# kchmck/p25rx

Measured on AMD Instinct MI355X. Metric: IQ Msamples/s through FM-demod+C4FM slice, higher is better.
Workload: dtype f32

## Files before the change

### p25rx_amd/csrc/p25fe_api.hip

```cpp
#include "p25fe_kernels.hip"

#include <hip/hip_ext.h>
#include <math.h>
#include <stdio.h>
#include <stdlib.h>
#include <string.h>

#include <algorithm>
#include <array>
#include <chrono>
#include <new>
#include <utility>
#include <string>
#include <vector>

#include "p25fe_jit.h"

using namespace p25k;

namespace {

constexpr size_t BBPAD = 256;
constexpr size_t SHARD_HALO = 2560;
static_assert(SHARD_HALO >= (size_t)(DEC * (PLPAD + CLK_L + 160) + TMAX) && 160 >= TMAX + TMAX - 1 && SHARD_HALO % 8 == 0, "shard halo");
// ... 204 lines not shown
    bool on = false;
    int level = 1;
    std::vector<hipEvent_t> ev;
    std::vector<uint8_t> mask;
    uint64_t calls = 0, seq = 0;
    int slot = -1;
    void begin()
    {
        if (on && level == 3 && (seq++ % PROF_SAMPLE) != 0) { slot = -1; return; }
        slot = on ? (int)(calls++ % PROF_RING) : -1;
        if (slot >= 0) mask[(size_t)slot] = 0;
    }
    void end() { slot = -1; }
    void mark(int idx, hipStream_t st, bool ext_events)
    {
        if (slot < 0 || (idx > 1 && level != 1) || (idx <= 1 && ext_events)) return;
        if (hipEventRecord(ev[(size_t)slot * 5 + idx], st) == hipSuccess) mask[(size_t)slot] |= (uint8_t)(1u << idx);
    }
    void k1_events(bool ext_events, hipEvent_t* e0, hipEvent_t* e1)
    {
        *e0 = *e1 = nullptr;
        if (slot < 0 || !ext_events) return;
        *e0 = ev[(size_t)slot * 5 + 0]; *e1 = ev[(size_t)slot * 5 + 1];
        mask[(size_t)slot] |= 3u;
    }
};

constexpr size_t WIN_PARITY = 2, WIN_RING = 4;
struct WinSlot {
    hipEvent_t h2d_begin = nullptr, h2d_end = nullptr;
    hipEvent_t comp_begin = nullptr, comp_end = nullptr;
    hipEvent_t on_host = nullptr;
    std::array<hipEvent_t*, 5> all() { return {&h2d_begin, &h2d_end, &comp_begin, &comp_end, &on_host}; }
};
struct Windows {
    DevBuf buf[WIN_PARITY], dib[WIN_PARITY], res, anc;
    PinBuf stage[WIN_PARITY], out;
    hipStream_t cs = nullptr, os = nullptr;
    WinSlot slot[WIN_RING];
    WinSlot& of(size_t k) { return slot[k % WIN_RING]; }
    hipError_t ensure()
    {
        if (cs) return hipSuccess;
        hipError_t e = hipStreamCreateWithFlags(&cs, hipStreamNonBlocking);
        if (e == hipSuccess) e = hipStreamCreateWithFlags(&os, hipStreamNonBlocking);
        for (WinSlot& s : slot) for (hipEvent_t* x : s.all()) if (e == hipSuccess) e = hipEventCreate(x);
        return e;
    }
};

}

struct p25fe {
    p25fe_config_t cfg;
    int C = 1, n_cu = 256;
    Taps taps;
    int k1_p = 5;
    int variant = P25FE_VARIANT_BUILTIN;
    bool dflt = true;
    bool long_taps = false;
    int phase = P25FE_DECIM_PHASE;
    int n_avg = BOX;
    bool u8_lut_mode = false;
    float u8_scale = 0.0f, u8_offset = 0.0f;
    int track = 0;
    bool causal_ok = false;
    long look = 0;
    bool ext_events = true;
    int rx_cus = 0;
    int run_depth = 2;
    int sh_depth = MAX_LANES;

    int last_hip = 0;
    DevBuf d_taps;
    hipModule_t jit_mod = nullptr;
    hipFunction_t jit_fn[2][3] = {{nullptr, nullptr, nullptr}, {nullptr, nullptr, nullptr}};
    hipStream_t stream = nullptr, rx_stream = nullptr;
    const long* rs_idx = nullptr; size_t rs_n = 0, rs_stride = 0;
    Lane lanes[MAX_LANES];
    int cur = 0, lane_q[MAX_LANES - 1] = {1, 2, 3};
    Lane& lane() { return lanes[cur]; }
    RxScratch& rx() { return lanes[cur].s; }
    const RxScratch& rx() const { return lanes[cur].s; }
    DevBuf power_partial, chunk_cnt, evrec, evnext, evoff;
    unsigned long long ev_seq = 0;
    PinBuf hin, hbb, hout;
    unsigned chunk_seq = 0;
    Windows win; StreamState state; Prof prof; ShardCtx sh;
};

struct PlanarGeo {
    size_t n_tiles, n_blocks;
    explicit PlanarGeo(size_t n_bb)
    {
        n_tiles = (n_bb + TS - 1) / TS;
        if (n_tiles == 0) n_tiles = 1;
        n_blocks = (size_t)TWORDS * n_tiles + 6;
    }
    size_t floats() const { return n_blocks * PL_BLK; }
    size_t words() const { return n_blocks * SPS; }
};

constexpr size_t MAX_RANGE_BB = (size_t)0x7ff00000u * 10u;
static inline bool position_refused(uint64_t pos) { return pos >= P25FE_MAX_POSITION; }

struct Resolved {
    Taps taps;
    bool long_taps;
    bool lut_affine;
    float u8_scale, u8_offset;
    bool dflt;
};

static inline bool finite_f(float v) { return v - v == 0.0f; }
static inline bool same_bits(float a, float b) { return memcmp(&a, &b, sizeof a) == 0; }

static bool lut_is_affine(const float* lut, float sc, float of)
{
    for (int b = 0; b < 256; ++b)
        if (!same_bits(lut[b], fmaf((float)b, sc, of))) return false;
    return true;
}

static int resolve_config(const p25fe_config_t* cfg, Resolved* r)
{
    if (cfg->abi_version != P25FE_ABI_VERSION || cfg->n_decim_taps < 1 || cfg->n_decim_taps > P25FE_MAX_TAPS || cfg->n_chan_taps < 1 ||
        cfg->n_chan_taps > P25FE_MAX_TAPS || (cfg->symbol_clock != P25FE_CLOCK_FIXED && cfg->symbol_clock != P25FE_CLOCK_TRACKING && cfg->symbol_clock != P25FE_CLOCK_TRACKING_RESLICE &&
         cfg->symbol_clock != (P25FE_CLOCK_TRACKING_RESLICE | P25FE_CLOCK_CAUSAL_OK)) ||
        cfg->specialize < P25FE_SPECIALIZE_OFF || cfg->specialize > P25FE_SPECIALIZE_FORCE || cfg->decim_phase < 0 || cfg->decim_phase >= DEC ||
        cfg->n_avg_taps < 1 || cfg->n_avg_taps > P25FE_MAX_TAPS)
        return P25FE_ERR_ARG;
    memset(&r->taps, 0, sizeof r->taps);
    r->taps.n_avg = cfg->n_avg_taps;
    r->taps.avg_uniform = 1;
    for (int k = 0; k < cfg->n_avg_taps; ++k) {
        if (!finite_f(cfg->avg_taps[k])) return P25FE_ERR_ARG;
        r->taps.avg[k] = cfg->avg_taps[k];
        if (!same_bits(cfg->avg_taps[k], cfg->avg_taps[0])) r->taps.avg_uniform = 0;
    }
    for (int k = 0; k < cfg->n_decim_taps; ++k) { if (!finite_f(cfg->decim_taps[k])) return P25FE_ERR_ARG; r->taps.dec[k] = cfg->decim_taps[k]; }
    for (int k = 0; k < cfg->n_chan_taps; ++k) { if (!finite_f(cfg->chan_taps[k])) return P25FE_ERR_ARG; r->taps.ch[k] = cfg->chan_taps[k]; }
    r->long_taps = cfg->n_decim_taps > P25FE_T1 || cfg->n_chan_taps > P25FE_T2;
    if (cfg->fm_gain != 0.0f) {
        if (!finite_f(cfg->fm_gain)) return P25FE_ERR_ARG;
        r->taps.fm_gain = cfg->fm_gain;
    } else {
        if (cfg->fm_deviation_hz == 0 || cfg->fm_sample_rate_hz == 0) return P25FE_ERR_ARG;
        r->taps.fm_gain = (float)((double)cfg->fm_sample_rate_hz / (2.0 * M_PI * (double)cfg->fm_deviation_hz));
    }
    if (cfg->u8_lut_valid) {
        for (int b = 0; b < 256; ++b) { if (!finite_f(cfg->u8_lut[b])) return P25FE_ERR_ARG; r->taps.lut[b] = cfg->u8_lut[b]; }
        const float* L = r->taps.lut;
        const float cand[3][2] = {{cfg->u8_scale, cfg->u8_offset}, {L[1] - L[0], L[0]},
                                  {(float)(((double)L[255] - (double)L[0]) / 255.0), L[0]}};
        r->lut_affine = false;
        for (int c = 0; c < 3 && !r->lut_affine; ++c)
            if (finite_f(cand[c][0]) && finite_f(cand[c][1]) && lut_is_affine(L, cand[c][0], cand[c][1])) {
                r->lut_affine = true; r->u8_scale = cand[c][0]; r->u8_offset = cand[c][1];
            }
        if (!r->lut_affine) r->u8_scale = r->u8_offset = 0.0f;
    } else {
        if (!finite_f(cfg->u8_scale) || !finite_f(cfg->u8_offset)) return P25FE_ERR_ARG;
        r->lut_affine = true; r->u8_scale = cfg->u8_scale; r->u8_offset = cfg->u8_offset;
        for (int b = 0; b < 256; ++b) r->taps.lut[b] = fmaf((float)b, cfg->u8_scale, cfg->u8_offset);
    }
    Taps def;
    memset(&def, 0, sizeof def);
// ... 583 lines not shown

static int launch_planarize(p25fe_t* h, const float* d_bb, size_t bb_stride, size_t n_hist_bb, size_t n_bb, hipStream_t st)
{
    const PlanarGeo g(n_bb);
    PlanarizeArgs a;
    a.bb = d_bb; a.bb_stride = (long)bb_stride; a.n_hist = (long)n_hist_bb; a.n = (long)n_bb;
    a.f = h->rx().pl_f.get(); a.f_ch = (long)g.floats();
    a.bits = h->rx().pl_bits.get(); a.bits_ch = (long)g.words(); a.n_blocks = (long)g.n_blocks;
    a.shift = (int)h->look;
    hipLaunchKernelGGL(k_planarize, dim3((unsigned)((g.n_blocks + 1) / 2), (unsigned)h->C), dim3(WV * SPS), 0, st, a);
    HIPCHK(h, hipGetLastError());
    return P25FE_OK;
}

static int launch_detect(p25fe_t* h, const RecvCall& rc)
{
    DetArgs d;
    d.head_flag = nullptr; d.head_seq = 0u; d.head_tile_max = -1; d.head_err = nullptr;
    if (rc.wait_head) {
        d.head_flag = h->sh.flag.as<unsigned>(); d.head_seq = h->sh.seq; d.head_tile_max = h->sh.head_tile_max;
        d.head_err = h->sh.flag.as<unsigned>() + SH_FLAG_ERR;
    }
    view_planes(h, rc.range, &d); view_tiles(h, &d); view_general(h, &d);
    d.n_tiles = n_tiles_of(rc.range); d.opt = rc.opt;
    const dim3 grid((unsigned)d.n_tiles, (unsigned)h->C);
    if (rc.gen) hipLaunchKernelGGL(k_detect<true>, grid, dim3(WV), 0, rc.stream, d);
    else hipLaunchKernelGGL(k_detect<false>, grid, dim3(WV), 0, rc.stream, d);
    HIPCHK(h, hipGetLastError());
    return P25FE_OK;
}

enum ScanStep { SCAN_WHOLE, SCAN_RANGE, SCAN_TILES_G };
static int launch_scan(p25fe_t* h, const RecvCall& rc, ScanStep step, hipEvent_t ev_done)
{
    const dim3 grid = step == SCAN_RANGE ? dim3((unsigned)h->C) : dim3((unsigned)n_groups_of(n_tiles_of(rc.range)), (unsigned)h->C);
    if (rc.gen) {
        ScanArgsG c;
        view_scan(h, rc, &c);
        c.gsum = h->rx().gsum.get(); c.outs = h->rx().gouts.get(); c.gsg = h->rx().gsg.get(); c.gpg = h->rx().gpg.get();
        c.track = h->track;
        launch_ev(step == SCAN_WHOLE ? k_scan_tiles_g : step == SCAN_RANGE ? k_range_scan_g : k_scan_g_groups, grid, dim3(WV), 0, rc.stream,
                  nullptr, ev_done, c);
    } else {
        ScanArgs c;
        view_scan(h, rc, &c);
        c.tsum = h->rx().tsum.get(); c.outs = h->rx().outs.get(); c.gagg = h->rx().gagg.get(); c.gpre = h->rx().gpre.get();
        launch_ev(step == SCAN_WHOLE ? k_scan_tiles : k_range_scan, grid, dim3(WV), 0, rc.stream, nullptr, ev_done, c);
    }
    HIPCHK(h, hipGetLastError());
    return P25FE_OK;
}

static int launch_slice(p25fe_t* h, const RecvCall& rc)
{
    SliceArgs l;
    view_planes(h, rc.range, &l); view_tiles(h, &l); view_dest(rc.range, rc.dest, &l);
    l.n_tiles = n_tiles_of(rc.range); l.outs = h->rx().outs.get(); l.gpre = h->rx().gpre.get(); l.dibits2 = rc.dest.dibits2;
    if (rc.fix) l.fix = *rc.fix; else memset(&l.fix, 0, sizeof l.fix);
    launch_ev(k_slice, dim3((unsigned)l.n_tiles + (rc.fix ? 1u : 0u), (unsigned)h->C), dim3(WV), 0, rc.stream, nullptr, rc.ev_done, l);
    HIPCHK(h, hipGetLastError());
    return P25FE_OK;
}

static int launch_slice_g(p25fe_t* h, const RecvCall& rc)
{
    SliceArgsG l;
    view_planes(h, rc.range, &l); view_general(h, &l); view_dest(rc.range, rc.dest, &l);
    l.n_tiles = n_tiles_of(rc.range); l.outs = h->rx().gouts.get(); l.recs = h->rx().recs.get();
    l.track = h->track; l.dibits2 = rc.dest.dibits2;
    launch_ev(k_slice_g, dim3((unsigned)l.n_tiles, (unsigned)h->C), dim3(WV), 0, rc.stream, nullptr, rc.ev_done, l);
    HIPCHK(h, hipGetLastError());
    return P25FE_OK;
}

static int launch_slice_by_detection(p25fe_t* h, const RecvCall& rc)
{
    const size_t C = (size_t)h->C, n_bb = rc.range.n_bb;
    const int n_tiles = n_tiles_of(rc.range);
    hipStream_t st = rc.stream;
    size_t cap_ev = (size_t)n_tiles * EVCAP;
    const size_t bound = n_bb / (size_t)(W + 1) + (size_t)n_tiles + 8;
    if (bound < cap_ev) cap_ev = bound;
    const size_t stride = cap_ev + 2;
    HIPCHK(h, h->evrec.ensure(C * stride * sizeof(EvRec)));
    HIPCHK(h, h->evoff.ensure(C * (stride + 1) * sizeof(unsigned long long)));
    {
        const void* before = h->evnext.p;
        HIPCHK(h, h->evnext.ensure(C * stride * sizeof(EvNext)));
        if (h->evnext.p != before) HIPCHK(h, hipMemsetAsync(h->evnext.p, 0, h->evnext.cap, st));
    }
    EvArgs e;
    view_planes(h, rc.range, &e); view_general(h, &e); view_dest(rc.range, rc.dest, &e);
    e.n_tiles = n_tiles; e.outs = h->rx().gouts.get();
    e.rec = h->evrec.as<EvRec>(); e.nxt = h->evnext.as<EvNext>(); e.off = h->evoff.as<unsigned long long>();
    e.ev_stride = (long)stride; e.seq = ++h->ev_seq; e.result = rc.dest.result;
    hipLaunchKernelGGL(k_ev_collect, dim3((unsigned)n_tiles, (unsigned)h->C), dim3(WV), 0, st, e);
    HIPCHK(h, hipGetLastError());
    hipLaunchKernelGGL(k_ev_count, dim3((unsigned)(n_tiles < 1024 ? n_tiles : 1024), (unsigned)h->C), dim3(WV), 0, st, e);
    HIPCHK(h, hipGetLastError());
    hipLaunchKernelGGL(k_ev_scan, dim3((unsigned)h->C), dim3(WV), 0, st, e);
    HIPCHK(h, hipGetLastError());
    const size_t max_dibits = n_bb / (SPS - 1) + (size_t)n_tiles + 64;
    const size_t lim = rc.dest.dibit_stride < max_dibits ? rc.dest.dibit_stride : max_dibits;
    launch_ev(k_ev_slice, dim3((unsigned)((lim + WV * 4 - 1) / (WV * 4)), (unsigned)h->C), dim3(WV), 0, st, nullptr, rc.ev_done, e);
    HIPCHK(h, hipGetLastError());
    return P25FE_OK;
}

static int launch_recv(p25fe_t* h, const RecvCall& rc)
{
    const int n_tiles = n_tiles_of(rc.range);
    const bool detect = rc.detect && n_tiles != 0, slice = rc.slice && n_tiles != 0, scan = rc.fix == nullptr;
    hipStream_t st = rc.stream;
    int e = detect ? launch_detect(h, rc) : P25FE_OK;
    if (e) return e;
    h->prof.mark(2, st, h->ext_events);
    if (scan && (e = launch_scan(h, rc, detect ? SCAN_WHOLE : SCAN_RANGE, slice ? nullptr : rc.ev_done)) != P25FE_OK) return e;
    h->prof.mark(3, st, h->ext_events);
    if (slice) {
        if (!rc.gen) e = launch_slice(h, rc);
        else if ((e = launch_scan(h, rc, SCAN_TILES_G, nullptr)) == P25FE_OK) e = rc.reslice ? launch_slice_by_detection(h, rc) : launch_slice_g(h, rc);
        if (e) return e;
    }
    if (rc.ev_done && !scan && !slice) HIPCHK(h, hipEventRecord(rc.ev_done, st));
    h->prof.mark(4, st, h->ext_events);
    return P25FE_OK;
}

static int launch_k1_planar(p25fe_t* h, K1Launch& k, hipEvent_t k1_done, hipStream_t waiter)
{
    h->prof.mark(0, k.stream, h->ext_events);
    bool attached = false;
    if (p25fe_n_baseband_h(h, k.abs0, k.n)) {
        h->prof.k1_events(h->ext_events, &k.ev0, &k.ev1);
        if (k1_done && h->ext_events) {
            if (k.ev1) k1_done = k.ev1;
            else k.ev1 = k1_done;
            attached = true;
        }
        k.planar = true;
        if (int rc = launch_k1(h, k)) return rc;
    }
    if (k1_done) {
        if (!attached) HIPCHK(h, hipEventRecord(k1_done, k.stream));
        HIPCHK(h, hipStreamWaitEvent(waiter, k1_done, 0));
    }
    return P25FE_OK;
}

static int launch_planar_recv(p25fe_t* h, K1Launch& k, const RecvCall& rc, hipEvent_t k1_done = nullptr)
{
    if (int e = launch_k1_planar(h, k, k1_done, rc.stream)) return e;
    if (rc.range.n_bb) h->prof.mark(1, k.stream, h->ext_events);
    return launch_recv(h, rc);
}

static inline bool piecewise_refused(const p25fe_t* h) { return h->track == P25FE_CLOCK_TRACKING_RESLICE && !h->causal_ok; }

static WideConv wide_conv_of(const p25fe_t* h)
{
    WideConv cv;
    cv.scale = h->u8_scale; cv.offset = h->u8_offset;
    cv.lut = h->u8_lut_mode ? h->d_taps.as<Taps>()->lut : nullptr;
    return cv;
}
static inline bool wide_fmt_known(int fmt) { return fmt == P25FE_FMT_CF32 || fmt == P25FE_FMT_S16 || fmt == P25FE_FMT_U8; }
static inline int wide_o0(uint64_t abs0) { return (int)((PD - 1 + PD - abs0 % PD) % PD); }

static int launch_k0(p25fe_t* h, const void* d_iq, int fmt, size_t ch_stride, size_t n_hist, size_t n, uint64_t abs0,
                     float* d_out, size_t out_stride, hipStream_t st)
{
    if (!d_iq || !d_out || position_refused(abs0)) return P25FE_ERR_ARG;
    if ((reinterpret_cast<uintptr_t>(d_iq) & 15u) != 0 || (h->C > 1 && ch_stride % fmt_stride_unit(fmt) != 0)) return P25FE_ERR_ARG;
    HIPCHK(h, hipSetDevice(h->cfg.device));
    const size_t n_out = p25fe_n_predecim(abs0, n);
    if (n_out == 0) return P25FE_OK;
    K0Args a;
    a.x = static_cast<const float*>(d_iq); a.ch_stride = (long)ch_stride; a.n_hist = (long)n_hist; a.n_new = (long)n;
    a.o0 = wide_o0(abs0);
    a.y = d_out; a.y_stride = (long)out_stride; a.n_out = (long)n_out;
    const size_t per_wg = (size_t)K0_SUB * K0_SUBS;
    const dim3 grid((unsigned)((n_out + per_wg - 1) / per_wg), (unsigned)h->C);
    const WideConv cv = wide_conv_of(h);
    if (fmt == P25FE_FMT_CF32) hipLaunchKernelGGL(k_predecim, grid, dim3(WV), 0, st, a);
    else if (fmt == P25FE_FMT_S16) hipLaunchKernelGGL((k_predecim_fmt<P25FE_FMT_S16, false>), grid, dim3(WV), 0, st, a, cv);
    else if (cv.lut) hipLaunchKernelGGL((k_predecim_fmt<P25FE_FMT_U8, true>), grid, dim3(WV), 0, st, a, cv);
    else hipLaunchKernelGGL((k_predecim_fmt<P25FE_FMT_U8, false>), grid, dim3(WV), 0, st, a, cv);
// ... 1571 lines not shown
```

### p25rx_amd/csrc/p25fe_recv.hip

```cpp
#ifndef __HIPCC_RTC__
#include <hip/hip_runtime.h>
#include <stdint.h>
#endif

namespace p25k {

constexpr int W = P25FE_PEAK_W;
constexpr int SPS = P25FE_SPS;
constexpr int NSYN = P25FE_SYNC_DIBITS;
constexpr int SYNC_SPAN = P25FE_SYNC_SPAN;
constexpr int HIST_BB = SYNC_SPAN + 2 * W;
static_assert(SPS == SPS_ && PLPAD >= HIST_BB + P25FE_CLK_LOOKAHEAD, "planar layout matches the receiver");

constexpr int TSYM = 768;
constexpr int TS = TSYM * SPS;
constexpr int TWORDS = TSYM / 32;
constexpr int EVCAP = TS / (W + 1) + 8;
constexpr unsigned SYNC_NEG_MASK = ~P25FE_SYNC_SIGN_MASK & 0xffffffu;
constexpr int SCREEN_MAX_MISMATCH = 4;

struct Planar {
    const float* f;
    long f_ch;
    const uint32_t* bits;
// ... 1432 lines not shown
                } else {
                    const int e = (int)(i - T0) + PL_BLK;
                    if (track) {
                        const float* w = CI + 4 * (q & (P25FE_CLK_PHASES - 1));
                        v = w[0] * sample_at(e - 1);
                        v = __builtin_fmaf(w[1], sample_at(e), v);
                        v = __builtin_fmaf(w[2], sample_at(e + 1), v);
                        v = __builtin_fmaf(w[3], sample_at(e + 2), v);
                    } else {
                        v = sample_at(e);
                    }
                }
                if (rank >= 0 && rank + idx < room) {
                    const unsigned char db = slice_dibit(v, h, m, l);
                    dst[idx] = db;
                    if (out2) out2[rank + idx] = db;
                }
            }
        }
        return count;
    };

    int rank = 0;
    if (valid) rank += emit(so.s, so.D, so.N, T0, g.pre_end1 ? T0 + (long)g.pre_end1 - 1 : TE, hi, mid, lo, 0);
    unsigned eg = 0u, eg_prev = 0u;
    int ev_prev = 0;
    for (int k = 0; k < n_ev; ++k) {
        const int evk = ev_at(k, eg);
        const long ek = T0 + evk, sk = ek - W;
        int D, N;
        if (k == 0) clock_period(track, ((g.n_det_flags >> 16) & G_FIRST_TRACKS) && valid, so.s, so.f, sk, frac3(eg >> 16), D, N);
        else clock_period(track, ((eg >> 15) & 1u) != 0, T0 + ev_prev - W, frac3(eg_prev >> 16), sk, frac3(eg >> 16), D, N);
        float h, m, l;
        if (k < EVTHR_N) {
            h = rdl_f(el.th, 3 * k); m = rdl_f(el.th, 3 * k + 1); l = rdl_f(el.th, 3 * k + 2);
        } else {
            float v[NSYN];
            sync_gather(f, t0 + evk - W + PLPAD, v);
            sync_thresholds(v, h, m, l);
        }
        if (lane == 0 && a.sync_pos && (long)(so.event_off + k) < a.sync_stride) {
            a.sync_pos[(size_t)ch * a.sync_stride + so.event_off + k] = sk;
            a.sync_dibit[(size_t)ch * a.sync_stride + so.event_off + k] = so.dibit_off + (unsigned long long)rank;
        }
        rank += emit(sk, D, N, ek + 1, T0 + (long)(eg & 0x7fffu), h, m, l, rank);
        ev_prev = evk; eg_prev = eg;
    }
}
__global__ __launch_bounds__(WV, 4) void k_slice_g(SliceArgsG a) { slice_g_item(a, (int)blockIdx.x, (int)blockIdx.y); }
#endif

struct EvRec {
    long s;
    long g_lo, g_hi;
    int Db, Nb;
    int D2, N2;
    unsigned flags;
    float hi, mid, lo;
    int pad_;
};
static_assert(sizeof(EvRec) == 64, "EvRec layout");
struct EvNext { long pos; unsigned long long seq; };
constexpr unsigned EV_USABLE = 1u, EV_OPEN = 2u, EV_VALID = 4u;
__host__ __device__ inline long clock_J_off(long x, int D, int N, int off)
{
    const long num = x * (long)N - (long)off - 1;
    return num < 0 ? 0 : num / (long)D;
}

struct EvArgs {
    Planar pl;
    long n, abs0;
    int n_tiles;
    const ScanOutG* outs;
    const TileSumG* gsum;
    const uint16_t* evl;
    const uint32_t* evg;
    const float* evthr;
    const p25fe_anchor_t* anchor_in;
    EvRec* rec;
    EvNext* nxt;
    unsigned long long* off;
    long ev_stride;
    unsigned long long seq;
    p25fe_result_t* result;
    uint8_t* dibits;
    long dibit_stride;
    int64_t* sync_pos;
    uint64_t* sync_dibit;
    long sync_stride;
};

#ifndef P25FE_JIT
__device__ __forceinline__ void ev_collect_item(const EvArgs& a, const int tile, const int ch)
{
    const int lane = threadIdx.x;
    const long t0 = (long)tile * TS;
    const int tn = a.n - t0 < TS ? (int)(a.n - t0) : TS;
    const ScanOutG so = a.outs[(size_t)ch * a.n_tiles + tile];
    const TileSumG g = a.gsum[(size_t)ch * a.n_tiles + tile];
    const int n_ev = (int)(g.n_det_flags & 0xffffu);
    const long T0 = a.abs0 + t0;
    EvRec* rec = a.rec + (size_t)ch * a.ev_stride;
    EvNext* nxt = a.nxt + (size_t)ch * a.ev_stride;
    p25fe_anchor_t Ain;
    Ain.valid = 0; Ain.s = 0; Ain.hi = Ain.mid = Ain.lo = 0.f; Ain.period_d = SPS; Ain.period_n = 1;
    if (a.anchor_in) Ain = a.anchor_in[ch];
    const bool carry_valid = so.src >= 0 || (so.src == -1 && Ain.valid != 0);
    if (tile == 0 && lane == 0) {
        EvRec r;
        r.s = Ain.s; r.g_lo = a.abs0; r.g_hi = a.abs0 + a.n;
        const bool ok = clock_plausible(Ain.period_d, Ain.period_n);
        r.Db = ok ? Ain.period_d : SPS; r.Nb = ok ? Ain.period_n : 1; r.D2 = r.Db; r.N2 = r.Nb;
        r.flags = EV_USABLE | EV_OPEN | (Ain.valid ? EV_VALID : 0u);
        r.hi = Ain.hi; r.mid = Ain.mid; r.lo = Ain.lo; r.pad_ = 0;
        rec[0] = r;
    }
    if (!g.pre_end1) return;
    if (lane == 0 && carry_valid) {
        EvNext x; x.pos = T0 + (long)g.pre_end1 - 1; x.seq = a.seq;
        nxt[so.event_off] = x;
    }
    if (n_ev == 0) return;
    const uint16_t* evl = a.evl + ((size_t)ch * a.n_tiles + tile) * EVCAP;
    const uint32_t* evg = a.evg + ((size_t)ch * a.n_tiles + tile) * EVCAP;
    const float* f = a.pl.f + (size_t)ch * a.pl.f_ch;
    const float* eth = a.evthr + ((size_t)ch * a.n_tiles + tile) * (EVTHR_N * 3);
    for (int k0 = 0; k0 < n_ev; k0 += WV) {
        const int k = k0 + lane;
        if (k < n_ev) {
            const unsigned eg = evg[k];
            const long ek = T0 + evl[k], sk = ek - W;
            const unsigned eg_p = k ? evg[k - 1] : 0u;
            const long s_p = k ? T0 + evl[k - 1] - W : 0;
            EvRec r;
            bool us;
            if (k == 0) clock_period(true, ((g.n_det_flags >> 16) & G_FIRST_TRACKS) && carry_valid, so.s, so.f, sk, frac3(eg >> 16), r.Db, r.Nb, &us);
            else clock_period(true, ((eg >> 15) & 1u) != 0, s_p, frac3(eg_p >> 16), sk, frac3(eg >> 16), r.Db, r.Nb, &us);
            r.s = sk; r.g_lo = ek + 1; r.g_hi = T0 + (long)(eg & 0x7fffu);
            r.D2 = r.Db; r.N2 = r.Nb;
            r.flags = EV_VALID | (us ? EV_USABLE : 0u) | ((k == n_ev - 1 && (int)(eg & 0x7fffu) == tn) ? EV_OPEN : 0u) | (((eg >> 16) & 7u) << 8);
            r.hi = r.mid = r.lo = 0.f; r.pad_ = 0;
            EvRec* dst = rec + 1 + so.event_off + k;
            if (k < EVTHR_N) {
                r.hi = eth[3 * k]; r.mid = eth[3 * k + 1]; r.lo = eth[3 * k + 2];
                *dst = r;
            } else {
                dst->s = r.s; dst->g_lo = r.g_lo; dst->g_hi = r.g_hi; dst->Db = r.Db; dst->Nb = r.Nb; dst->D2 = r.D2; dst->N2 = r.N2;
                dst->flags = r.flags; dst->pad_ = 0;
            }
        }
    }
    for (int k = EVTHR_N; k < n_ev; ++k) {
        float v[NSYN], h, m, l;
        sync_gather(f, t0 + (int)evl[k] - W + PLPAD, v);
        sync_thresholds(v, h, m, l);
        if (lane == 0) { EvRec* r = rec + 1 + so.event_off + k; r->hi = h; r->mid = m; r->lo = l; }
    }
}
__global__ __launch_bounds__(WV, 4) void k_ev_collect(EvArgs a) { ev_collect_item(a, (int)blockIdx.x, (int)blockIdx.y); }

__global__ __launch_bounds__(WV, 4) void k_ev_count(EvArgs a)
{
    const int lane = threadIdx.x, ch = blockIdx.y;
    EvRec* rec = a.rec + (size_t)ch * a.ev_stride;
    const EvNext* nxt = a.nxt + (size_t)ch * a.ev_stride;
    const long n_e = (long)a.result[ch].n_sync + 1;
    const long range_end = a.abs0 + a.n;
    for (long e = (long)blockIdx.x * WV + lane; e < n_e; e += (long)gridDim.x * WV) {
        const EvRec r = rec[e];
        unsigned cnt = 0u;
        long jlo = 1;
        if (r.flags & EV_VALID) {
            int D = r.Db, N = r.Nb;
            if (!(r.flags & EV_USABLE) && e + 1 < n_e) {
                if (rec[e + 1].flags & EV_USABLE) { D = rec[e + 1].Db; N = rec[e + 1].Nb; }
            }
            long ghi = r.g_hi;
            if (r.flags & EV_OPEN) {
                const EvNext x = nxt[e];
                ghi = x.seq == a.seq ? x.pos : range_end;
            }
            if (N == 1) { D *= 4; N = 4; }
            const int off = frac3(r.flags >> 8) * (N / 4);
            long glo = r.g_lo < r.s + W + 1 ? r.s + W + 1 : r.g_lo;
            const long j0 = clock_J_off(glo - r.s, D, N, off);
            long c = ghi > glo ? clock_J_off(ghi - r.s, D, N, off) - j0 : 0;
            cnt = (unsigned)(c < 0 ? 0 : (c > 0x7fffffffL ? 0x7fffffffL : c));
            jlo = j0 + 1;
            rec[e].D2 = D; rec[e].N2 = N; rec[e].g_hi = ghi;
        }
        rec[e].g_lo = jlo;
        rec[e].pad_ = (int)cnt;
    }
}

constexpr int EVC_PER = 16;
__global__ __launch_bounds__(WV) void k_ev_scan(EvArgs a)
{
    const int lane = threadIdx.x, ch = blockIdx.x;
    const EvRec* rec = a.rec + (size_t)ch * a.ev_stride;
    unsigned long long* off = a.off + (size_t)ch * (a.ev_stride + 1);
    const long n_e = (long)a.result[ch].n_sync + 1;
    unsigned long long c_base = 0ull;
    for (long c0 = 0; c0 < n_e; c0 += (long)WV * EVC_PER) {
        unsigned cnt[EVC_PER];
        unsigned long long mine = 0;
#pragma unroll
        for (int q = 0; q < EVC_PER; ++q) {
            const long e = c0 + (long)lane * EVC_PER + q;
            cnt[q] = e < n_e ? (unsigned)rec[e].pad_ : 0u;
            mine += cnt[q];
        }
        const unsigned long long incl = wave_incl_sum64(mine, lane);
        unsigned long long o = c_base + incl - mine;
#pragma unroll
        for (int q = 0; q < EVC_PER; ++q) {
            const long e = c0 + (long)lane * EVC_PER + q;
            if (e < n_e) {
                off[e] = o;
                if (e >= 1 && a.sync_pos && e - 1 < a.sync_stride) {
                    a.sync_pos[(size_t)ch * a.sync_stride + e - 1] = rec[e].s;
                    a.sync_dibit[(size_t)ch * a.sync_stride + e - 1] = o;
                }
                o += cnt[q];
            }
        }
        c_base += __shfl(incl, WV - 1, 64);
    }
    if (lane == 0) {
        off[n_e] = c_base;
        p25fe_result_t r = a.result[ch];
        r.n_dibits = c_base;
        r.n_dibits_after_first = n_e >= 2 ? c_base - off[1] : 0;
        a.result[ch] = r;
    }
}

__global__ __launch_bounds__(WV, 4) void k_ev_slice(EvArgs a)
{
    __shared__ float CI[P25FE_CLK_PHASES * 4];
    const int lane = threadIdx.x, ch = blockIdx.y;
    const EvRec* rec = a.rec + (size_t)ch * a.ev_stride;
    const unsigned long long* off = a.off + (size_t)ch * (a.ev_stride + 1);
    const long n_e = (long)a.result[ch].n_sync + 1;
    const unsigned long long total = off[n_e];
    const unsigned long long g0 = (unsigned long long)blockIdx.x * (WV * 4);
    if (g0 >= total) return;
    for (int k = lane; k < P25FE_CLK_PHASES * 4; k += WV) CI[k] = P25FE_CLK_INTERP[k];
    phase_sync();
    const float* f = a.pl.f + (size_t)ch * a.pl.f_ch;
    uint8_t* out = a.dibits + (size_t)ch * a.dibit_stride;
    long e0 = 0;
    {
        long hi_ = n_e;
        while (hi_ - e0 > 1) {
            const long mid_ = (e0 + hi_) >> 1;
            if (off[mid_] <= g0) e0 = mid_; else hi_ = mid_;
        }
    }
    long lo_ = e0;
#pragma unroll
    for (int q = 0; q < 4; ++q) {
        const unsigned long long gi = g0 + (unsigned long long)(q * WV + lane);
        if (gi < total && (long)gi < a.dibit_stride) {
            while (lo_ + 1 < n_e && off[lo_ + 1] <= gi) ++lo_;
            const EvRec r = rec[lo_];
            const long j = r.g_lo + (long)(gi - off[lo_]);
            const long num = j * (long)r.D2 + (long)(frac3(r.flags >> 8) * (r.N2 / 4));
            const long qu = num / r.N2;
            const long i = r.s + qu;
            const int ph = (int)((((unsigned)(num - qu * r.N2) * (unsigned)P25FE_CLK_PHASES) / (unsigned)r.N2) & (unsigned)(P25FE_CLK_PHASES - 1));
            if (i < a.abs0 || i >= a.abs0 + a.n) { out[gi] = 0; continue; }
            const long p = i - a.abs0 + PLPAD;
            float b[4];
#pragma unroll
            for (int tq = 0; tq < 4; ++tq) {
                const long pp = p - 1 + tq;
                const long sy = pp / SPS;
                b[tq] = f[planar_index(sy, (int)(pp - sy * SPS))];
            }
            const float* w = CI + 4 * ph;
            float v = w[0] * b[0];
            v = __builtin_fmaf(w[1], b[1], v);
            v = __builtin_fmaf(w[2], b[2], v);
            v = __builtin_fmaf(w[3], b[3], v);
            out[gi] = slice_dibit(v, r.hi, r.mid, r.lo);
        }
    }
}
#endif

constexpr int TAILN = 256;

struct ChunkRecvArgs {
    Planar pl;
    long n;
    long abs0;
    TileRec* recs;
    unsigned long long* tsum;
    uint16_t* evl;
    float* evthr;
    const p25fe_anchor_t* anchor_in;
    p25fe_result_t* result;
    uint8_t* dibits;
    long dibit_stride;
    int64_t* sync_pos;
    uint64_t* sync_dibit;
    long sync_stride;
    float* tail;
    int look;
    unsigned long long n_baseband;
    unsigned* done;
    unsigned seq;
};

__device__ __forceinline__ void wave_global_sync() { __builtin_amdgcn_fence(__ATOMIC_SEQ_CST, "workgroup"); }

__device__ __forceinline__ void tail_extract(const ChunkRecvArgs& c, const int ch)
{
    if (!c.tail) return;
    const float* f = c.pl.f + (size_t)ch * c.pl.f_ch;
    for (int j = (int)threadIdx.x; j < TAILN; j += WV) {
        const long m = c.n - TAILN + j;
        if (m >= -(long)(HIST_BB + c.look)) {
            const long pp = m + c.look + PLPAD;
            const long sy = pp / SPS;
            c.tail[(size_t)ch * TAILN + j] = f[planar_index(sy, (int)(pp - sy * SPS))];
        }
    }
}
#ifndef P25FE_JIT
__global__ __launch_bounds__(WV) void k_tail_extract(ChunkRecvArgs c) { tail_extract(c, (int)blockIdx.x); }
#endif

__device__ __forceinline__ void recv_one_tile(const ChunkRecvArgs& c, const int ch)
{
    const int lane = threadIdx.x;
    DetArgs d;
    d.pl = c.pl; d.n = c.n; d.abs0 = c.abs0; d.n_tiles = 1;
    d.recs = c.recs; d.tsum = c.tsum; d.evl = c.evl; d.evthr = c.evthr;
    d.opt.track = 0; d.opt.n_resync = 0; d.opt.resync = nullptr; d.opt.resync_stride = 0; d.gsum = nullptr; d.evg = nullptr;
    d.head_flag = nullptr; d.head_seq = 0u; d.head_tile_max = -1; d.head_err = nullptr;
    detect_tile<false>(d, 0, ch);
    wave_global_sync();
    const TileRec rc = c.recs[ch];
    const unsigned long long u = c.tsum[ch];
    p25fe_anchor_t A = c.anchor_in[ch];
    if (!clock_plausible(A.period_d, A.period_n)) { A.period_d = SPS; A.period_n = 1; }
    const bool own = rc.n_events > 0;
    const unsigned long long pre = A.valid ? (unsigned long long)count_instants(A.s, c.abs0, own ? rc.first_event + 1 : c.abs0 + c.n) : 0ull;
    if (lane == 0) {
        p25fe_result_t r;
        r.n_baseband = c.n_baseband;
        r.n_dibits = pre + (own ? (unsigned long long)rc.post_count : 0ull);
        r.n_sync = own ? (unsigned long long)rc.n_events : 0ull;
        p25fe_anchor_t out = A;
        if (own) { out.valid = 1; out.s = rc.last_s; out.hi = rc.hi; out.mid = rc.mid; out.lo = rc.lo; out.period_d = SPS; out.period_n = 1; }
        r.anchor_out = out;
        r.first_event = own ? rc.first_event : -1;
        r.n_dibits_after_first = own ? (unsigned long long)rc.post_count : 0ull;
        r.carry_end = own ? rc.first_event + 1 : -1;
        r.first_seg_end = -1; r.flags = 0u; r.reserved = 0u;
        c.result[ch] = r;
    }
    SliceArgs l;
    l.pl = c.pl; l.n = c.n; l.abs0 = c.abs0; l.n_tiles = 1;
    l.outs = nullptr; l.recs = c.recs; l.tsum = c.tsum; l.evl = c.evl; l.evthr = c.evthr; l.anchor_in = c.anchor_in;
    l.dibits = c.dibits; l.dibit_stride = c.dibit_stride;
    l.sync_pos = (c.sync_pos && c.sync_dibit) ? c.sync_pos : nullptr; l.sync_dibit = c.sync_dibit; l.sync_stride = c.sync_stride;
    l.dibits2 = nullptr; l.fix.summ = nullptr; l.gpre = nullptr;
// ... 76 lines not shown
```

Baseline: 544,900.

## Precompute block-to-event index in scan and slice runs per event with 32-bit math

The scan kernel now also writes a coarse block index mapping each group of output dibits to its starting event, so slice blocks look up their event without a binary search over offsets. The slice kernel finds the events covering its block with wave ballots, then processes each event's run with 32-bit divides and direct planar addressing. Blocks with many events, or indices that fall outside safe ranges, take the old wide 64-bit path. The count kernel's grid is also resized from the input length instead of the tile count. This adds an extra buffer and several code paths, so there is a risk of subtle indexing errors.

Measured after the change: 541,100. Within noise of the previous version (-0.7%).

```diff
diff --git a/p25rx_amd/csrc/p25fe_api.hip b/p25rx_amd/csrc/p25fe_api.hip
--- a/p25rx_amd/csrc/p25fe_api.hip
+++ b/p25rx_amd/csrc/p25fe_api.hip
@@ -310,7 +310,7 @@
     Lane& lane() { return lanes[cur]; }
     RxScratch& rx() { return lanes[cur].s; }
     const RxScratch& rx() const { return lanes[cur].s; }
-    DevBuf power_partial, chunk_cnt, evrec, evnext, evoff;
+    DevBuf power_partial, chunk_cnt, evrec, evnext, evoff, evblk;
     unsigned long long ev_seq = 0;
     PinBuf hin, hbb, hout;
     unsigned chunk_seq = 0;
@@ -1060,6 +1060,10 @@
     const size_t bound = n_bb / (size_t)(W + 1) + (size_t)n_tiles + 8;
     if (bound < cap_ev) cap_ev = bound;
     const size_t stride = cap_ev + 2;
+    const size_t max_dibits = n_bb / (SPS - 1) + (size_t)n_tiles + 64;
+    const size_t lim = rc.dest.dibit_stride < max_dibits ? rc.dest.dibit_stride : max_dibits;
+    const size_t n_blk = (lim + EVB - 1) / EVB;
+    const size_t blk_stride = (2 + (max_dibits + EVG - 1) / EVG + 1) & ~(size_t)1;
     HIPCHK(h, h->evrec.ensure(C * stride * sizeof(EvRec)));
     HIPCHK(h, h->evoff.ensure(C * (stride + 1) * sizeof(unsigned long long)));
     {
@@ -1067,20 +1071,23 @@
         HIPCHK(h, h->evnext.ensure(C * stride * sizeof(EvNext)));
         if (h->evnext.p != before) HIPCHK(h, hipMemsetAsync(h->evnext.p, 0, h->evnext.cap, st));
     }
+    HIPCHK(h, h->evblk.ensure(C * blk_stride * sizeof(unsigned)));
     EvArgs e;
     view_planes(h, rc.range, &e); view_general(h, &e); view_dest(rc.range, rc.dest, &e);
     e.n_tiles = n_tiles; e.outs = h->rx().gouts.get();
     e.rec = h->evrec.as<EvRec>(); e.nxt = h->evnext.as<EvNext>(); e.off = h->evoff.as<unsigned long long>();
     e.ev_stride = (long)stride; e.seq = ++h->ev_seq; e.result = rc.dest.result;
+    e.blk = h->evblk.as<unsigned>(); e.blk_stride = (long)blk_stride; e.n_blk = (long)((lim + EVG - 1) / EVG);
     hipLaunchKernelGGL(k_ev_collect, dim3((unsigned)n_tiles, (unsigned)h->C), dim3(WV), 0, st, e);
     HIPCHK(h, hipGetLastError());
-    hipLaunchKernelGGL(k_ev_count, dim3((unsigned)(n_tiles < 1024 ? n_tiles : 1024), (unsigned)h->C), dim3(WV), 0, st, e);
+    size_t n_cnt = (n_bb / (size_t)(864 * SPS) + 2 + WV - 1) / WV;
+    if (n_cnt > 1024) n_cnt = 1024;
+    if (n_cnt > (stride + WV - 1) / WV) n_cnt = (stride + WV - 1) / WV;
+    hipLaunchKernelGGL(k_ev_count, dim3((unsigned)n_cnt, (unsigned)h->C), dim3(WV), 0, st, e);
     HIPCHK(h, hipGetLastError());
     hipLaunchKernelGGL(k_ev_scan, dim3((unsigned)h->C), dim3(WV), 0, st, e);
     HIPCHK(h, hipGetLastError());
-    const size_t max_dibits = n_bb / (SPS - 1) + (size_t)n_tiles + 64;
-    const size_t lim = rc.dest.dibit_stride < max_dibits ? rc.dest.dibit_stride : max_dibits;
-    launch_ev(k_ev_slice, dim3((unsigned)((lim + WV * 4 - 1) / (WV * 4)), (unsigned)h->C), dim3(WV), 0, st, nullptr, rc.ev_done, e);
+    launch_ev(k_ev_slice, dim3((unsigned)n_blk, (unsigned)h->C), dim3(WV), 0, st, nullptr, rc.ev_done, e);
     HIPCHK(h, hipGetLastError());
     return P25FE_OK;
 }
diff --git a/p25rx_amd/csrc/p25fe_recv.hip b/p25rx_amd/csrc/p25fe_recv.hip
--- a/p25rx_amd/csrc/p25fe_recv.hip
+++ b/p25rx_amd/csrc/p25fe_recv.hip
@@ -1538,6 +1538,9 @@
     EvNext* nxt;
     unsigned long long* off;
     long ev_stride;
+    unsigned* blk;
+    long blk_stride;
+    long n_blk;
     unsigned long long seq;
     p25fe_result_t* result;
     uint8_t* dibits;
@@ -1616,6 +1619,59 @@
 }
 __global__ __launch_bounds__(WV, 4) void k_ev_collect(EvArgs a) { ev_collect_item(a, (int)blockIdx.x, (int)blockIdx.y); }
 
+constexpr int EVB = WV * 4;
+constexpr int EVG = 16 * EVB;
+constexpr int EVC_PER = 16;
+
+__global__ __launch_bounds__(WV) void k_ev_scan(EvArgs a)
+{
+    const int lane = threadIdx.x, ch = blockIdx.x;
+    const long n_e = (long)a.result[ch].n_sync + 1;
+    const EvRec* rec = a.rec + (size_t)ch * a.ev_stride;
+    unsigned long long* off = a.off + (size_t)ch * (a.ev_stride + 1);
+    unsigned* blkc = a.blk + (size_t)ch * a.blk_stride;
+    unsigned* blk = blkc + 2;
+    const bool lists = a.sync_pos != nullptr;
+    unsigned long long c_base = 0ull, off1 = 0ull;
+    for (long c0 = 0; c0 < n_e; c0 += (long)WV * EVC_PER) {
+        unsigned cnt[EVC_PER];
+        unsigned long long mine = 0;
+#pragma unroll
+        for (int q = 0; q < EVC_PER; ++q) {
+            const long e = c0 + (long)lane * EVC_PER + q;
+            cnt[q] = e < n_e ? (unsigned)rec[e].pad_ : 0u;
+            mine += cnt[q];
+        }
+        const unsigned long long incl = wave_incl_sum64(mine, lane);
+        unsigned long long o = c_base + incl - mine;
+        if (c0 == 0) off1 = __shfl(o + cnt[0], 0, 64);
+        long nb = (long)((o + (EVG - 1)) / EVG);
+        unsigned long long nd = (unsigned long long)nb * EVG;
+#pragma unroll
+        for (int q = 0; q < EVC_PER; ++q) {
+            const long e = c0 + (long)lane * EVC_PER + q;
+            if (e < n_e) {
+                off[e] = o;
+                if (e >= 1 && lists && e - 1 < a.sync_stride) {
+                    a.sync_pos[(size_t)ch * a.sync_stride + e - 1] = rec[e].s;
+                    a.sync_dibit[(size_t)ch * a.sync_stride + e - 1] = o;
+                }
+            }
+            o += cnt[q];
+            while (nd < o && nb < a.n_blk) { blk[nb] = (unsigned)e; ++nb; nd += EVG; }
+        }
+        c_base += __shfl(incl, WV - 1, 64);
+    }
+    if (lane == 0) {
+        off[n_e] = c_base;
+        *reinterpret_cast<unsigned long long*>(blkc) = c_base;
+        p25fe_result_t r = a.result[ch];
+        r.n_dibits = c_base;
+        r.n_dibits_after_first = n_e >= 2 ? c_base - off1 : 0;
+        a.result[ch] = r;
+    }
+}
+
 __global__ __launch_bounds__(WV, 4) void k_ev_count(EvArgs a)
 {
     const int lane = threadIdx.x, ch = blockIdx.y;
@@ -1651,98 +1707,129 @@
     }
 }
 
-constexpr int EVC_PER = 16;
-__global__ __launch_bounds__(WV) void k_ev_scan(EvArgs a)
-{
-    const int lane = threadIdx.x, ch = blockIdx.x;
-    const EvRec* rec = a.rec + (size_t)ch * a.ev_stride;
-    unsigned long long* off = a.off + (size_t)ch * (a.ev_stride + 1);
-    const long n_e = (long)a.result[ch].n_sync + 1;
-    unsigned long long c_base = 0ull;
-    for (long c0 = 0; c0 < n_e; c0 += (long)WV * EVC_PER) {
-        unsigned cnt[EVC_PER];
-        unsigned long long mine = 0;
+__device__ __forceinline__ unsigned char ev_dibit_wide(const EvArgs& a, const float* f, const long s, const int D2, const int N2, const unsigned flags,
+                                                       const float hi, const float mid, const float lo, const long j)
+{
+    const long num = j * (long)D2 + (long)(frac3(flags >> 8) * (N2 / 4));
+    const long qu = num / N2;
+    const long i = s + qu;
+    const int ph = (int)((((unsigned)(num - qu * N2) * (unsigned)P25FE_CLK_PHASES) / (unsigned)N2) & (unsigned)(P25FE_CLK_PHASES - 1));
+    if (i < a.abs0 || i >= a.abs0 + a.n) return 0;
+    const long p = i - a.abs0 + PLPAD;
+    float b[4];
 #pragma unroll
-        for (int q = 0; q < EVC_PER; ++q) {
-            const long e = c0 + (long)lane * EVC_PER + q;
-            cnt[q] = e < n_e ? (unsigned)rec[e].pad_ : 0u;
-            mine += cnt[q];
-        }
-        const unsigned long long incl = wave_incl_sum64(mine, lane);
-        unsigned long long o = c_base + incl - mine;
-#pragma unroll
-        for (int q = 0; q < EVC_PER; ++q) {
-            const long e = c0 + (long)lane * EVC_PER + q;
-            if (e < n_e) {
-                off[e] = o;
-                if (e >= 1 && a.sync_pos && e - 1 < a.sync_stride) {
-                    a.sync_pos[(size_t)ch * a.sync_stride + e - 1] = rec[e].s;
-                    a.sync_dibit[(size_t)ch * a.sync_stride + e - 1] = o;
-                }
-                o += cnt[q];
-            }
-        }
-        c_base += __shfl(incl, WV - 1, 64);
-    }
-    if (lane == 0) {
-        off[n_e] = c_base;
-        p25fe_result_t r = a.result[ch];
-        r.n_dibits = c_base;
-        r.n_dibits_after_first = n_e >= 2 ? c_base - off[1] : 0;
-        a.result[ch] = r;
-    }
-}
-
+    for (int tq = 0; tq < 4; ++tq) {
+        const long pp = p - 1 + tq;
+        const long sy = pp / SPS;
+        b[tq] = f[planar_index(sy, (int)(pp - sy * SPS))];
+    }
+    const float* w = P25FE_CLK_INTERP + 4 * ph;
+    float v = w[0] * b[0];
+    v = __builtin_fmaf(w[1], b[1], v);
+    v = __builtin_fmaf(w[2], b[2], v);
+    v = __builtin_fmaf(w[3], b[3], v);
+    return slice_dibit(v, hi, mid, lo);
+}
+
+constexpr int EV_RUNS = 4;
 __global__ __launch_bounds__(WV, 4) void k_ev_slice(EvArgs a)
 {
-    __shared__ float CI[P25FE_CLK_PHASES * 4];
     const int lane = threadIdx.x, ch = blockIdx.y;
     const EvRec* rec = a.rec + (size_t)ch * a.ev_stride;
     const unsigned long long* off = a.off + (size_t)ch * (a.ev_stride + 1);
+    const unsigned* blkc = a.blk + (size_t)ch * a.blk_stride;
+    const unsigned long long total = *reinterpret_cast<const unsigned long long*>(blkc);
+    const unsigned long long g0 = (unsigned long long)blockIdx.x * EVB;
+    const long ei = (long)blkc[2 + g0 / EVG];
     const long n_e = (long)a.result[ch].n_sync + 1;
-    const unsigned long long total = off[n_e];
-    const unsigned long long g0 = (unsigned long long)blockIdx.x * (WV * 4);
-    if (g0 >= total) return;
-    for (int k = lane; k < P25FE_CLK_PHASES * 4; k += WV) CI[k] = P25FE_CLK_INTERP[k];
-    phase_sync();
+    unsigned long long gend = g0 + EVB < total ? g0 + EVB : total;
+    const unsigned long long room = a.dibit_stride > 0 ? (unsigned long long)a.dibit_stride : 0ull;
+    if (gend > room) gend = room;
+    if ((g0 >= gend) | (ei >= n_e)) return;
     const float* f = a.pl.f + (size_t)ch * a.pl.f_ch;
     uint8_t* out = a.dibits + (size_t)ch * a.dibit_stride;
-    long e0 = 0;
-    {
-        long hi_ = n_e;
-        while (hi_ - e0 > 1) {
-            const long mid_ = (e0 + hi_) >> 1;
-            if (off[mid_] <= g0) e0 = mid_; else hi_ = mid_;
-        }
-    }
-    long lo_ = e0;
-#pragma unroll
-    for (int q = 0; q < 4; ++q) {
-        const unsigned long long gi = g0 + (unsigned long long)(q * WV + lane);
-        if (gi < total && (long)gi < a.dibit_stride) {
-            while (lo_ + 1 < n_e && off[lo_ + 1] <= gi) ++lo_;
-            const EvRec r = rec[lo_];
-            const long j = r.g_lo + (long)(gi - off[lo_]);
-            const long num = j * (long)r.D2 + (long)(frac3(r.flags >> 8) * (r.N2 / 4));
-            const long qu = num / r.N2;
-            const long i = r.s + qu;
-            const int ph = (int)((((unsigned)(num - qu * r.N2) * (unsigned)P25FE_CLK_PHASES) / (unsigned)r.N2) & (unsigned)(P25FE_CLK_PHASES - 1));
-            if (i < a.abs0 || i >= a.abs0 + a.n) { out[gi] = 0; continue; }
-            const long p = i - a.abs0 + PLPAD;
-            float b[4];
-#pragma unroll
-            for (int tq = 0; tq < 4; ++tq) {
-                const long pp = p - 1 + tq;
-                const long sy = pp / SPS;
-                b[tq] = f[planar_index(sy, (int)(pp - sy * SPS))];
-            }
-            const float* w = CI + 4 * ph;
-            float v = w[0] * b[0];
-            v = __builtin_fmaf(w[1], b[1], v);
-            v = __builtin_fmaf(w[2], b[2], v);
-            v = __builtin_fmaf(w[3], b[3], v);
-            out[gi] = slice_dibit(v, r.hi, r.mid, r.lo);
-        }
+    const long ew = ei + lane;
+    const unsigned long long ov = ew <= n_e ? off[ew] : total;
+    const int es = __builtin_popcountll(__ballot(ew < n_e && ov <= g0)) - 1;
+    const int m = __builtin_popcountll(__ballot(ew < n_e && ov > g0 && ov < gend));
+    if (es < 0 || es + EV_RUNS >= WV || m >= EV_RUNS) {
+        long lo_ = ei + (es < 0 ? 0 : es);
+        if (es == WV - 1) {
+            long hi_ = n_e;
+            while (hi_ - lo_ > 1) {
+                const long mid_ = (lo_ + hi_) >> 1;
+                if (off[mid_] <= g0) lo_ = mid_; else hi_ = mid_;
+            }
+        }
+#pragma unroll 1
+        for (int q = 0; q < EVB / WV; ++q) {
+            const unsigned long long gi = g0 + (unsigned long long)(q * WV + lane);
+            if (gi < gend) {
+                while (lo_ + 1 < n_e && off[lo_ + 1] <= gi) ++lo_;
+                const EvRec r = rec[lo_];
+                out[gi] = ev_dibit_wide(a, f, r.s, r.D2, r.N2, r.flags, r.hi, r.mid, r.lo, r.g_lo + (long)(gi - off[lo_]));
+            }
+        }
+        return;
+    }
+    const long e0 = ei + es;
+    EvRec rk = rec[e0];
+    EvRec rn = rec[e0 + 1 < n_e ? e0 + 1 : e0];
+#pragma unroll 1
+    for (int k = 0; ; ) {
+        const unsigned long long o_k = (unsigned long long)rdl_l((long)ov, es + k);
+        const unsigned long long a_k = o_k > g0 ? o_k : g0;
+        const unsigned long long b_k = k == m ? gend : (unsigned long long)rdl_l((long)ov, es + k + 1);
+        if (b_k > a_k) {
+            const int nrun = (int)(b_k - a_k);
+            const long j0 = rk.g_lo + (long)(a_k - o_k);
+            const int D2 = rk.D2, N2 = rk.N2;
+            const long num0 = j0 * (long)D2 + (long)(frac3(rk.flags >> 8) * (N2 / 4));
+            bool narrow = false;
+            long i0 = 0;
+            unsigned r0 = 0u;
+            if (N2 >= 4 && N2 < (1 << 26) && D2 > 0 && (long)D2 <= 16L * N2 && num0 >= 0 && num0 < (1L << 62)) {
+                const long q0 = num0 / (long)N2;
+                const long rr = num0 - q0 * (long)N2;
+                i0 = rk.s + q0;
+                r0 = (unsigned)rr;
+                narrow = (unsigned long long)rr + (unsigned long long)(nrun - 1) * (unsigned long long)D2 < (1ull << 32)
+                         && i0 >= a.abs0 && i0 < a.abs0 + a.n;
+            }
+            if (narrow) {
+                const long pb = i0 - a.abs0 + (PLPAD - 1);
+                const long B0 = pb / PL_BLK;
+                const int eb = (int)(pb - B0 * PL_BLK);
+                const float* fb = f + B0 * (long)PL_BLK;
+                auto sample_at = [&](int e) -> float {
+                    const int sy = e / SPS, r = e - sy * SPS;
+                    return fb[(sy >> 5) * PL_BLK + r * 32 + (sy & 31)];
+                };
+                const long i_end = a.abs0 + a.n;
+                for (int idx = lane; idx < nrun; idx += WV) {
+                    const unsigned t = r0 + (unsigned)idx * (unsigned)D2;
+                    const unsigned qu = t / (unsigned)N2;
+                    const int ph = (int)((((t - qu * (unsigned)N2) * (unsigned)P25FE_CLK_PHASES) / (unsigned)N2) & (unsigned)(P25FE_CLK_PHASES - 1));
+                    unsigned char db = 0;
+                    if (i0 + (long)qu < i_end) {
+                        const int e = eb + (int)qu;
+                        const float* w = P25FE_CLK_INTERP + 4 * ph;
+                        float v = w[0] * sample_at(e);
+                        v = __builtin_fmaf(w[1], sample_at(e + 1), v);
+                        v = __builtin_fmaf(w[2], sample_at(e + 2), v);
+                        v = __builtin_fmaf(w[3], sample_at(e + 3), v);
+                        db = slice_dibit(v, rk.hi, rk.mid, rk.lo);
+                    }
+                    out[a_k + (unsigned long long)idx] = db;
+                }
+            } else {
+                for (int idx = lane; idx < nrun; idx += WV)
+                    out[a_k + (unsigned long long)idx] = ev_dibit_wide(a, f, rk.s, D2, N2, rk.flags, rk.hi, rk.mid, rk.lo, j0 + idx);
+            }
+        }
+        if (++k > m) break;
+        rk = rn;
+        if (k < m) rn = rec[e0 + k + 1];
     }
 }
 #endif
```
